# LiChaiUSTC/Speech-enhancement-based-on-a-maximum-likelihood-criterion

Hardware: AMD Instinct MI355X
Metric: training frames/sec (128-frame minibatch) (higher is better)
Workload: dtype f32

## Files before the change

### speech-enhancement-based-on-a-maximum-likelihood-criterion_amd/csrc/engine.hip

```cpp
#include <hip/hip_runtime.h>
#include <hip/hip_ext.h>

#include <dlfcn.h>
#include <math.h>
#include <stdarg.h>
#include <stdio.h>
#include <stdlib.h>
#include <string.h>

#include <algorithm>
#include <functional>
#include <mutex>
#include <string>
#include <vector>

#include "../../include/mlggd.h"
#include "../host/errmodel.h"
#include "kernels.hip.h"
#include "spectral.hip.h"
#include "score.hip.h"
#include "stoi.hip.h"
#include "stoi_rule.h"
#include "live.hip.h"
#include "live_rule.h"
// ... 545 lines not shown
                gather_arm(e);
            ProfScope ps(e, KC_FWD, l);
            FwdArgs fa = fwd_args(e, l, e->Y[l]);
            if (fwd64_used(e, l)) {
                fa.n_tiles = Np / 64;
                fa.b_tiles = e->Bp / 64;
                fa.b_shift = log2_or_minus1(fa.b_tiles);
                const size_t lds = t64_lds_floats() * sizeof(float);
                if (l != e->L - 1 && relu) {
                    CHK(ensure_lds(e, k_fwd64<FWD_RELU>, lds));
                    launch_timed(e, k_fwd64<FWD_RELU>, dim3(fa.n_tiles * fa.b_tiles), dim3(256), lds, e->stream, fa);
                } else if (l != e->L - 1) {
                    CHK(ensure_lds(e, k_fwd64<FWD_SIGMOID>, lds));
                    launch_timed(e, k_fwd64<FWD_SIGMOID>, dim3(fa.n_tiles * fa.b_tiles), dim3(256), lds, e->stream, fa);
                } else {
                    CHK(ensure_lds(e, k_fwd64<FWD_SLAB>, lds));
                    launch_timed(e, k_fwd64<FWD_SLAB>, dim3(fa.n_tiles * fa.b_tiles), dim3(256), lds, e->stream, fa);
                }
            } else if (l != e->L - 1) {
                long long *st = stamps_for(e, KC_FWD, l, n_tiles * b_tiles);
#define LAUNCH_FWD(NW, PIPE)                                                                                \
    {                                                                                                       \
        const size_t lds = fwd_lds_floats<NW, PIPE>() * sizeof(float);                                      \
        if (relu) {                                                                                         \
            CHK(ensure_lds(e, k_fwd<FWD_RELU, NW, PIPE>, lds));                                             \
            launch_timed(e, k_fwd<FWD_RELU, NW, PIPE>, dim3(n_tiles * b_tiles), dim3(64 * NW), lds, e->stream, fa, st); \
        } else {                                                                                            \
            CHK(ensure_lds(e, k_fwd<FWD_SIGMOID, NW, PIPE>, lds));                                          \
            launch_timed(e, k_fwd<FWD_SIGMOID, NW, PIPE>, dim3(n_tiles * b_tiles), dim3(64 * NW), lds, e->stream, fa, st); \
        }                                                                                                   \
    }
                if (e->fwd_nw == 16) LAUNCH_FWD(16, 0)
                else if (e->fwd_nw == 8 && e->fwd_pipe == 4) LAUNCH_FWD(8, 4)
                else if (e->fwd_nw == 8 && e->fwd_pipe) LAUNCH_FWD(8, 1)
                else if (e->fwd_nw == 8) LAUNCH_FWD(8, 0)
                else if (e->fwd_pipe == 4) LAUNCH_FWD(4, 4)
                else if (e->fwd_pipe) LAUNCH_FWD(4, 1)
                else LAUNCH_FWD(4, 0)
#undef LAUNCH_FWD
            } else {
                const int nwg = n_tiles * b_tiles * e->S_out;
                if (e->fwd_pipe == 4) {
                    const size_t lds = fwd_lds_floats<4, 4>() * sizeof(float);
                    CHK(ensure_lds(e, k_fwd<FWD_SLAB, 4, 4>, lds));
                    launch_timed(e, k_fwd<FWD_SLAB, 4, 4>, dim3(nwg), dim3(256), lds, e->stream, fa, (long long *)nullptr);
                } else {
                    const size_t lds = fwd_lds_floats<4, 1>() * sizeof(float);
                    launch_timed(e, k_fwd<FWD_SLAB, 4, 1>, dim3(nwg), dim3(256), lds, e->stream, fa, (long long *)nullptr);
                }
            }
        }
        CHK(launch_check("k_fwd"));
        if (cvscale) {
            const float keep = 1.0f - ((l == 1) ? e->cfg.visible_omit : e->cfg.hid_omit);
            hipLaunchKernelGGL(k_scale, dim3(1024), dim3(256), 0, e->stream, e->W[l], (size_t)Kp * Np, 1.0f / keep);
        }
        if (drop && l != e->L - 1) CHK(run_dropout(e, l, nullptr));
        if ((gather_flags & GATHER_HIDDEN_EACH) && l < e->L - 1) {
            CHK(gather_begin_armed(e));
            CHK(exchange_y(e, l, e->Y[l], nullptr));
            CHK(gather_end(e));
        }
// ... 51 lines not shown
    for (int j = 0; j < J.njobs && j < DWP_MAXJOBS; j++) {
        const DwpArgs &s = J.job[j];
        DwpArgs &a = key.job[j];
        a.Yrow = s.Yrow; a.dEdX = s.dEdX; a.Wt = s.Wt; a.delta = s.delta; a.G = s.G;
        a.bias = s.bias; a.dbias = s.dbias; a.gb = s.gb;
        a.ldA = s.ldA; a.K = s.K; a.N = s.N; a.Kp = s.Kp; a.Np = s.Np; a.n_wg = s.n_wg; a.ntiles = s.ntiles;
        a.k_first = s.k_first; a.wd_off = s.wd_off; a.do_bias = s.do_bias; a.k_base = s.k_base;
        key.tile_end[j] = J.tile_end[j];
    }
    key.njobs = J.njobs;
    key.total = J.total;
    for (const auto &t : e->dwp_tables)
        if (t.fused == fused && t.grid == grid && memcmp(&t.key, &key, sizeof(key)) == 0) {
            *out = t.dev;
            return MLGGD_OK;
        }
    if (e->dwp_tables.size() >= 64)
        return fail(MLGGD_ERR_STATE, "dW tile table: %zu launch plans cached and still missing -- plan key unstable",
                    e->dwp_tables.size());
    std::vector<DwpDesc> recs((size_t)J.total + 2 * (size_t)grid);
    size_t n = 0;
    for (int j = 0; j < J.njobs; j++) {
        const DwpArgs &a = J.job[j];
        for (int tl = 0; tl < a.ntiles; tl++, n++) {
            const int kt = a.k_first + tl / a.n_wg, nt = tl % a.n_wg;
            const int k0 = kt * 64, n0 = nt * 64;
            DwpDesc &d = recs[n];
            d.A = a.Yrow + (k0 - a.k_base);
            d.Bm = a.dEdX + n0;
            const size_t base = (size_t)k0 * a.Np + n0;
            int rows = a.K - k0;
            rows = rows < 0 ? 0 : rows > 64 ? 64 : rows;
            if (a.wd_off) {
                rows = 0;
                d.W = a.Wt;
                d.D = a.delta;
                d.szW = 0;
            } else {
                d.W = (fused ? a.Wt : a.G) + base;
                d.D = fused ? a.delta + base : nullptr;
                d.szW = (unsigned)(((size_t)a.Kp * a.Np - base) * sizeof(float));
            }
            const int colsw = a.Np - n0 < 64 ? a.Np - n0 : 64;
            int nbias = (a.do_bias && kt == 0) ? a.N - n0 : 0;
            nbias = nbias < 0 ? 0 : nbias > 64 ? 64 : nbias;
            d.bias = (fused ? a.bias : a.gb) + n0;
            d.dbias = fused ? a.dbias + n0 : nullptr;
            d.ldA = a.ldA;
            d.Np = a.Np;
            d.packed = (unsigned)rows | ((unsigned)colsw << 8) | ((unsigned)nbias << 16) | (1u << 24);
        }
    }
    if (n != (size_t)J.total) return fail(MLGGD_ERR_STATE, "dW tile table: %zu records for %d tiles", n, J.total);
    for (; n < recs.size(); n++) {
        DwpDesc &d = recs[n];
        d = recs[0];
        d.packed = 0;
        d.szW = 0;
    }
    mlggd_engine::DwpTable t;
    t.key = key;
    t.fused = fused;
    t.grid = grid;
    t.dev = nullptr;
// ... 26 lines not shown
        CHK(dwp_table(e, J, fused, grid, &table));
        unsigned nb;
        memcpy(&nb, &C.nf, sizeof(nb));
        if ((nb & 0x007FFFFFu) == 0u && C.nf >= 1.0f) {
            CHK(ensure_lds(e, k_dwp_bias<H, true>, lds));
            hipLaunchKernelGGL((k_dwp_bias<H, true>), dim3(grid), dim3(256), lds, st, table, J.total, C, (long long *)nullptr);
        } else {
            CHK(ensure_lds(e, k_dwp_bias<H, false>, lds));
            hipLaunchKernelGGL((k_dwp_bias<H, false>), dim3(grid), dim3(256), lds, st, table, J.total, C, (long long *)nullptr);
        }
        return launch_check("k_dwp_bias");
    }
    CHK(dwp_table(e, J, fused, grid, &table));
    if constexpr (H == 2 || H == 8) {
        if (e->stamp_class == KC_DW && e->stamp_layer == -1 && e->stamp_buf && fused && C.nf == 128.0f) {
            long long *sp = stamps_for(e, KC_DW, -1, 2 * grid);
            if (sp) {
                CHK(ensure_lds(e, k_dwp_phases<H>, lds));
                hipLaunchKernelGGL((k_dwp_phases<H>), dim3(grid), dim3(256), lds, st, table, J.total, C, sp);
                return launch_check("k_dwp_phases");
            }
        }
    }
    long long *stamps = stamps_for(e, KC_DW, stamp_layer, grid);
    if constexpr (H == 2) {
        static const int abl = getenv("MLGGD_DWP_ABLATE") ? atoi(getenv("MLGGD_DWP_ABLATE")) : 0;
        if (abl && fused) {
#define DWP_ABL(A_)                                                                                       \
    case A_:                                                                                              \
        CHK(ensure_lds(e, k_dwp_ablate<H, A_>, lds));                                                     \
        launch_timed(e, k_dwp_ablate<H, A_>, dim3(grid), dim3(256), lds, st, table, J.total, C, stamps);  \
        return launch_check("k_dwp_ablate");
            switch (abl) {
                DWP_ABL(1) DWP_ABL(2) DWP_ABL(3) DWP_ABL(4) DWP_ABL(7) DWP_ABL(15) DWP_ABL(31) DWP_ABL(63) DWP_ABL(16) DWP_ABL(48) DWP_ABL(256) DWP_ABL(512) DWP_ABL(576)
            default: return fail(MLGGD_ERR_ARG, "MLGGD_DWP_ABLATE=%d is not built", abl);
            }
#undef DWP_ABL
        }
    }
    unsigned nfbits;
    memcpy(&nfbits, &C.nf, sizeof(nfbits));
    const bool pow2 = (nfbits & 0x007FFFFFu) == 0u && C.nf >= 1.0f;
#define DWP_LAUNCH(FUSED_, POW2_)                                                                         \
    {                                                                                                     \
        CHK(ensure_lds(e, k_dwp<H, FUSED_, POW2_>, lds));                                                 \
        launch_timed(e, k_dwp<H, FUSED_, POW2_>, dim3(grid), dim3(256), lds, st, table, J.total, C, stamps); \
    }
    if (fused && pow2) DWP_LAUNCH(true, true)
    else if (fused) DWP_LAUNCH(true, false)
    else if (pow2) DWP_LAUNCH(false, true)
    else DWP_LAUNCH(false, false)
#undef DWP_LAUNCH
    return launch_check("k_dwp");
}
static bool dwp_usable(const mlggd_engine *e) {
    const int Hh = e->Bp / 64;
    return e->dw_persist && e->Bp % 64 == 0 && (Hh == 1 || Hh == 2 || Hh == 4 || Hh == 8);
}
static int launch_dwp(mlggd_engine *e, const DwpJobs &J, bool fused, hipStream_t st, int stamp_layer, int units = 0) {
    switch (units > 0 ? units : e->Bp / 64) {
    case 1: return launch_dwp_t<1>(e, J, fused, st, stamp_layer);
    case 2: return launch_dwp_t<2>(e, J, fused, st, stamp_layer);
    case 4: return launch_dwp_t<4>(e, J, fused, st, stamp_layer);
    case 8: return launch_dwp_t<8>(e, J, fused, st, stamp_layer);
    case 16: return launch_dwp_t<16>(e, J, fused, st, stamp_layer);
    default: return fail(MLGGD_ERR_STATE, "no dW kernel for %d units per tile", units);
    }
}

// ... 265 lines not shown
static int run_dx(mlggd_engine *e, int l) {
    const int Kp = e->lsp[l - 1], b_tiles = e->Bp / 32;
    const bool relu = e->cfg.activation == MLGGD_ACT_RELU;
    ProfScope ps(e, KC_DX, l);
    DxArgs xa = dx_args(e, l);
    if (dx64_used(e, l)) {
        xa.k_tiles = Kp / 64;
        xa.b_tiles = e->Bp / 64;
        xa.b_shift = log2_or_minus1(xa.b_tiles);
        const size_t lds = t64_lds_floats() * sizeof(float);
        if (relu) {
            CHK(ensure_lds(e, k_dx64<ACT_RELU>, lds));
            launch_timed(e, k_dx64<ACT_RELU>, dim3(xa.k_tiles * xa.b_tiles), dim3(256), lds, e->stream, xa);
        } else {
            CHK(ensure_lds(e, k_dx64<ACT_SIGMOID>, lds));
            launch_timed(e, k_dx64<ACT_SIGMOID>, dim3(xa.k_tiles * xa.b_tiles), dim3(256), lds, e->stream, xa);
        }
        return launch_check("k_dx64");
    }
    long long *st = stamps_for(e, KC_DX, l, (Kp / 32) * b_tiles);
#define LAUNCH_DX(NW, PIPE)                                                                                  \
    {                                                                                                        \
        const size_t lds = dx_lds_floats<NW, PIPE>() * sizeof(float);                                        \
        if (relu) {                                                                                          \
            CHK(ensure_lds(e, k_dx<NW, PIPE, ACT_RELU>, lds));                                               \
            launch_timed(e, k_dx<NW, PIPE, ACT_RELU>, dim3((Kp / 32) * b_tiles), dim3(64 * NW), lds, e->stream, xa, st); \
        } else {                                                                                             \
            CHK(ensure_lds(e, k_dx<NW, PIPE>, lds));                                                         \
            launch_timed(e, k_dx<NW, PIPE>, dim3((Kp / 32) * b_tiles), dim3(64 * NW), lds, e->stream, xa, st);  \
        }                                                                                                    \
    }
    const bool dma = e->dx_pipe == 4 && (Kp / 32) * b_tiles <= 256;
    if (e->dx_nw == 8 && e->dx_pipe) LAUNCH_DX(8, 1)
    else if (e->dx_nw == 8) LAUNCH_DX(8, 0)
    else if (dma) LAUNCH_DX(4, 4)
    else if (e->dx_pipe) LAUNCH_DX(4, 1)
    else LAUNCH_DX(4, 0)
#undef LAUNCH_DX
    return launch_check("k_dx");
}

static int launch_dw_layer(mlggd_engine *e, int l, const float *in_rows, bool fused, float nf, hipStream_t st) {
    const int Kp = e->lsp[l - 1], Np = e->lsp[l];
    const long tiles128 = (long)((Kp + 127) / 128) * ((Np + 127) / 128);
    const bool big = e->dw_tile == 0 ? tiles128 >= 192 : e->dw_tile == 2;
    ProfScope ps(e, KC_DW, l, st);
    if (dwp_usable(e)) return launch_dwp(e, dwp_jobs(e, l, l, in_rows, nf), fused, st, l);
    if (big) return launch_dw<2>(e, l, in_rows, fused, nf, st);
    return launch_dw<1>(e, l, in_rows, fused, nf, st);
}

static int launch_accum(float *dst, const float *a, const float *b, size_t n, hipStream_t st) {
    const size_t blocks = (n + 255) / 256;
    hipLaunchKernelGGL(k_accum, dim3((unsigned)(blocks > 2048 ? 2048 : blocks)), dim3(256), 0, st, dst, a, b, n);
    return launch_check("k_accum");
}

static size_t y_count(const mlggd_engine *e, int l) {
    return e->dp_a2a ? (size_t)e->world * e->Bp * e->shard_rows[l + 1] * 64 : (size_t)e->Bp * e->lsp[l];
}
static int keep_alloc(mlggd_engine *e) {
// ... 3281 lines not shown
```

### speech-enhancement-based-on-a-maximum-likelihood-criterion_amd/csrc/kernels.hip.h

```cpp
#pragma once
#include <hip/hip_runtime.h>
#include "nat_rule.h"

typedef float f32x16 __attribute__((ext_vector_type(16)));
typedef float f32x2 __attribute__((ext_vector_type(2)));

__device__ __forceinline__ f32x16 mfma32(float a, float b, f32x16 c) {
    return __builtin_amdgcn_mfma_f32_32x32x2f32(a, b, c, 0, 0, 0);
}
__device__ __forceinline__ int acc_row(int r, int lane) { return (r & 3) + 8 * (r >> 2) + 4 * (lane >> 5); }

__device__ __forceinline__ void divmod_by(int x, int d, int shift, int &q, int &r) {
    if (shift >= 0) {
        q = x >> shift;
        r = x & (d - 1);
    } else {
        q = (int)((unsigned)x / (unsigned)d);
        r = x - q * d;
    }
}
__device__ __forceinline__ void tile_of_block(int id, int u_tiles, int b_tiles, int b_shift, int &ut, int &bt, int map = 0) {
    if ((u_tiles & 7) == 0 && map != 2) {
        const int xcd = id & 7, slot = id >> 3;
        int q;
// ... 161 lines not shown
    const float *W, *Yt_in, *bias;
    float *Yt_out, *Y_out, *slab;
    int Kp, Np, Bp, N, n_tiles, b_tiles, S, map;
    int b_shift, s_shift;
    int yblk;
};
__device__ __forceinline__ size_t y_blocked_base(int u0, int yblk, int Bp) {
    const int blk = (int)((unsigned)u0 / (unsigned)yblk);
    return (size_t)blk * Bp * yblk + (u0 - blk * yblk);
}
template <int NW, int PIPE> constexpr int fwd_lds_floats() { return NW * (PIPE == 4 ? 4096 : 2048) + 32 * 36; }

template <int MODE, int NW, int PIPE = 1>
__device__ __forceinline__ void fwd_body(const FwdArgs &A, const int bid, float *smem, long long *stamps) {
    const float *__restrict__ W = A.W, *__restrict__ Yt_in = A.Yt_in, *__restrict__ bias = A.bias;
    float *__restrict__ Yt_out = A.Yt_out, *__restrict__ Y_out = A.Y_out, *__restrict__ slab = A.slab;
    const int Kp = A.Kp, Np = A.Np, Bp = A.Bp, N = A.N, n_tiles = A.n_tiles, b_tiles = A.b_tiles, S = A.S;
    float(*tileT)[36] = reinterpret_cast<float(*)[36]>(smem + NW * (PIPE == 4 ? 4096 : 2048));
    stamp(stamps, 0, bid);
    stamp_clk(stamps, 4, bid);
    const int tid = threadIdx.x, lane = tid & 63, wave = wave_id();
    const int i = lane & 31, h = lane >> 5;
    int id = bid, s = 0;
    if (MODE == FWD_SLAB) divmod_by(bid, S, A.s_shift, id, s);
    int nt, bt;
    tile_of_block(id, n_tiles, b_tiles, A.b_shift, nt, bt, A.map);
    const int n0 = nt * 32, b0 = bt * 32;

    const int P = Kp >> 1;
    const int slot = s * NW + wave, nslots = S * NW;
    int p0, p1;
    if (MODE == FWD_SLAB) {
        p0 = (int)((unsigned)(P * slot) / (unsigned)nslots);
        p1 = (int)((unsigned)(P * (slot + 1)) / (unsigned)nslots);
    } else {
        p0 = (int)((unsigned)(P * wave) / (unsigned)NW);
        p1 = (int)((unsigned)(P * (wave + 1)) / (unsigned)NW);
    }
    const int npairs = p1 - p0;
    const int nch = (npairs + 15) >> 4;

    const rsrc_t rW = make_rsrc(W, (size_t)Kp * Np * 4), rY = make_rsrc(Yt_in, (size_t)Kp * Bp * 4);
    const int r8 = lane >> 3, c4 = lane & 7;
    const int voW = (r8 * Np + n0 + 4 * c4) * 4, voY = (r8 * Bp + b0 + 4 * c4) * 4;
    float *stg = smem + wave * 2048;
    float *wdst = stg + r8 * 32 + 4 * c4;
// ... 830 lines not shown
    float *dbias;
    int ldA, Np;
    unsigned packed;
    unsigned szW;
};
static_assert(sizeof(DwpDesc) == 64, "four 16-byte quarters per record");
struct DwpRaw {
    unsigned w[16];
};
typedef unsigned u32x4 __attribute__((ext_vector_type(4)));
__device__ __forceinline__ DwpDesc dwp_decode(u32x4 v) {
    DwpRaw r;
#pragma unroll
    for (int q = 0; q < 4; q++)
#pragma unroll
        for (int c = 0; c < 4; c++) r.w[4 * q + c] = (unsigned)__builtin_amdgcn_readlane((int)v[c], q);
    return __builtin_bit_cast(DwpDesc, r);
}
struct DwpConst {
    int B;
    float nf, mom, lr, wc;
};

template <int H, bool FUSED, bool POW2, bool PHASES = false, int ABL = 0>
__device__ __forceinline__ void dwp_body(const DwpDesc *__restrict__ table, const int total, const DwpConst C, const int bid,
                                         const int nblocks, float *lds, long long *stamps) {
    stamp_clk(stamps, 0, bid);
    const int B = C.B;
    const float nf = C.nf, mom = C.mom, lr = C.lr, wc = C.wc;
    const float inv_nf = 1.0f / nf;
    constexpr int OOB = 0x7FFFFF00;
    const int tid = threadIdx.x, lane = tid & 63, wave = wave_id();
    const int i = lane & 31, h5 = lane >> 5;
    const int wm = wave >> 1, wn = wave & 1;
    const int scol = tid & 15, srow = tid >> 4;
    const int ec = lane & 7, er = lane >> 3;

    f32x16 acc, accp;
#pragma unroll
    for (int r = 0; r < 16; r++) acc[r] = accp[r] = 0.0f;
    float4 ra[4], rb[4];
    float4 pw0[4], pd0[4], pw1[4], pd1[4];
#pragma unroll
    for (int q = 0; q < 4; q++) pw1[q] = pd1[q] = make_float4(0.f, 0.f, 0.f, 0.f);
    float bsum = 0.0f, bsum_p = 0.0f;

    int t = bid;
    if (t >= total) return;
    const rsrc_t rT = make_rsrc(table, ((size_t)total + 2 * (size_t)nblocks) * sizeof(DwpDesc));
    const int voT = 16 * (lane & 3);
#define DWP_FETCH(TI) __builtin_bit_cast(u32x4, __builtin_amdgcn_raw_buffer_load_b128(rT, voT, (TI) * 64, 0))
    DwpDesc tc = dwp_decode(DWP_FETCH(t)), tn = dwp_decode(DWP_FETCH(t + nblocks)), tp = tc;
    tp.packed = 0;
    tp.szW = 0;
    u32x4 tnn_raw;

#define DWP_ROWS(T) ((int)((T).packed & 0xFFu))
#define DWP_COLS(T) ((int)(((T).packed >> 8) & 0xFFu))
#define DWP_NBIAS(T) ((int)(((T).packed >> 16) & 0xFFu))
#define DWP_SZAB(T) ((((T).packed >> 24) & 1u) ? 0x7FFFFFFFu : 0u)
#define DWP_DIVN(x) (POW2 ? (x) * inv_nf : (x) / nf)
#define DWP_DIVN2(x) (POW2 ? (x) * inv2 : (x) / nf2)
    const f32x2 mom2 = {mom, mom}, lr2 = {lr, lr}, wc2 = {wc, wc}, inv2 = {inv_nf, inv_nf}, nf2 = {nf, nf}, one2 = {1.0f, 1.0f};
#define DWP_OFF(T, IT)                                                                          \
    (((32 * wm + er + 8 * (IT)) < DWP_ROWS(T) && (32 * wn + 4 * ec) < DWP_COLS(T))               \
         ? ((32 * wm + er + 8 * (IT)) * T.Np + 32 * wn + 4 * ec) * 4                            \
         : OOB)
#define DWP_WRITE_UNIT(BUF)                                                                     \
    {                                                                                           \
        float *as = lds + (BUF)*8192, *bs = as + 4096;                                          \
        _Pragma("unroll") for (int q = 0; q < 4; q++) {                                         \
            *reinterpret_cast<float4 *>(as + (srow + 16 * q) * 64 + 4 * scol) = ra[q];          \
            *reinterpret_cast<float4 *>(bs + (srow + 16 * q) * 64 + 4 * scol) = rb[q];          \
        }                                                                                       \
    }
#define DWP_BIAS(BUF, HH)                                                                       \
    {                                                                                           \
        if (tid < DWP_NBIAS(tc)) {                                                              \
            const float *col = lds + (BUF)*8192 + 4096 + tid;                                   \
            int bend = B - 64 * (HH);                                                           \
            bend = bend < 64 ? bend : 64;                                                       \
            int b = 0;                                                                          \
            if ((HH) == 0 && bend > 0) {                                                        \
                bsum = col[0];                                                                  \
                b = 1;                                                                          \
            }                                                                                   \
            for (; b + 16 <= bend; b += 16) {                                                   \
                float v[16];                                                                    \
                _Pragma("unroll") for (int u = 0; u < 16; u++) v[u] = col[(b + u) * 64];        \
                _Pragma("unroll") for (int u = 0; u < 16; u++) bsum += v[u];                    \
            }                                                                                   \
            for (; b < bend; b++) bsum += col[b * 64];                                          \
        }                                                                                       \
    }
#define DWP_BIAS_UPDATE()                                                                       \
    {                                                                                           \
        if (tid < DWP_NBIAS(tp)) {                                                              \
            const rsrc_t rb_ = make_rsrc(tp.bias, 256), rdb_ = make_rsrc(tp.dbias, FUSED ? 256 : 0); \
            if (FUSED) {                                                                        \
                const float bv = bload(rb_, tid * 4, 0);                                        \
                const float d = mom * bload(rdb_, tid * 4, 0) - lr * (DWP_DIVN(bsum_p) + 0.0f * bv); \
                bstore1(d, rdb_, tid * 4);                                                      \
                bstore1(d + 1.0f * bv, rb_, tid * 4);                                           \
            } else {                                                                            \
                bstore1(bsum_p, rb_, tid * 4);                                                  \
            }                                                                                   \
        }                                                                                       \
    }
#define DWP_EPI_SCRATCH_WRITE(SB, R0, R1)                                                       \
    {                                                                                           \
        float *Tw = lds + (SB)*8192 + wave * 256;                                               \
        _Pragma("unroll") for (int r = (R0); r < (R1); r++) {                                   \
            const int kl = acc_row(r, lane);                                                    \
            Tw[(kl >> 3) * 1024 + ((kl >> 1) & 3) * 64 + (kl & 1) * 32 + i] = accp[r];          \
        }                                                                                       \
    }
#define DWP_EPI_SCRATCH_READ(SB, IT)                                                            \
    {                                                                                           \
        gq[IT] = *reinterpret_cast<const float4 *>(lds + (SB)*8192 + wave * 256 + (IT)*1024 + (er >> 1) * 64 + (er & 1) * 32 + 4 * ec); \
        asm volatile("" ::: "memory");                                                          \
    }
#define DWP_EPI_UPDATE(PW, PD, IT)                                                              \
    {                                                                                           \
        const float4 gv_ = gq[IT];                                                              \
        const int off = DWP_OFF(tp, IT);                                                        \
        if (FUSED && (ABL & 256)) {         \
            const float4 w = PW[IT];                                                            \
            float4 d = PD[IT];                                                                  \
            d.x = mom * d.x - lr * (DWP_DIVN(gv_.x) + wc * w.x);                                \
            d.y = mom * d.y - lr * (DWP_DIVN(gv_.y) + wc * w.y);                                \
            d.z = mom * d.z - lr * (DWP_DIVN(gv_.z) + wc * w.z);                                \
            d.w = mom * d.w - lr * (DWP_DIVN(gv_.w) + wc * w.w);                                \
            bstore4(d, rDp, off);                                                               \
            bstore4(make_float4(d.x + 1.0f * w.x, d.y + 1.0f * w.y, d.z + 1.0f * w.z, d.w + 1.0f * w.w), rWp, off); \
        } else if (FUSED) {  \
            const f32x2 w0 = {PW[IT].x, PW[IT].y}, w1 = {PW[IT].z, PW[IT].w};                   \
            f32x2 d0 = {PD[IT].x, PD[IT].y}, d1 = {PD[IT].z, PD[IT].w};                         \
            const f32x2 g0 = {gv_.x, gv_.y}, g1 = {gv_.z, gv_.w};                               \
            d0 = mom2 * d0 - lr2 * (DWP_DIVN2(g0) + wc2 * w0);                                  \
            d1 = mom2 * d1 - lr2 * (DWP_DIVN2(g1) + wc2 * w1);                                  \
            const f32x2 n0 = d0 + one2 * w0, n1 = d1 + one2 * w1;                               \
            bstore4(make_float4(d0.x, d0.y, d1.x, d1.y), rDp, off);                             \
            bstore4(make_float4(n0.x, n0.y, n1.x, n1.y), rWp, off);                             \
        } else {                                                                                \
            bstore4(gv_, rWp, off);                                                             \
        }                                                                                       \
    }
    long long ph_sum[5] = {0, 0, 0, 0, 0}, ph_last = 0;
#define DWP_PHASE(K)                                                                            \
    {                                                                                           \
        if (PHASES) {                                                                           \
            __builtin_amdgcn_sched_barrier(0);                                                  \
            const long long now_ = (long long)__builtin_amdgcn_s_memtime();                     \
            ph_sum[K] += now_ - ph_last;                                                        \
            ph_last = now_;                                                                     \
            __builtin_amdgcn_sched_barrier(0);                                                  \
        }                                                                                       \
    }
#define DWP_UNIT(HH, BUF, PW, PD)                                                               \
    {                                                                                           \
        const bool FIRSTU = (HH) == 0, LASTU = (HH) == H - 1;  \
        DWP_BIAS(BUF, HH)                                                                       \
        if (FIRSTU) DWP_BIAS_UPDATE()                                                           \
                                        \
        const rsrc_t rA_ = LASTU ? make_rsrc(tn.A, DWP_SZAB(tn)) : make_rsrc(tc.A, DWP_SZAB(tc)); \
        const rsrc_t rB_ = LASTU ? make_rsrc(tn.Bm, DWP_SZAB(tn)) : make_rsrc(tc.Bm, DWP_SZAB(tc)); \
        const int ldA_ = LASTU ? tn.ldA : tc.ldA, ldB_ = LASTU ? tn.Np : tc.Np;                 \
        const int row0_ = LASTU ? 0 : 64 * ((HH) + 1);                                          \
        const rsrc_t rWn = make_rsrc(tn.W, tn.szW), rDn = make_rsrc(tn.D, FUSED ? tn.szW : 0);  \
        const rsrc_t rWp = make_rsrc(tp.W, tp.szW), rDp = make_rsrc(tp.D, FUSED ? tp.szW : 0);  \
        const float *ap = lds + (BUF)*8192 + h5 * 64 + 32 * wm + i;                             \
        const float *bp = lds + (BUF)*8192 + 4096 + h5 * 64 + 32 * wn + i;                      \
        float fa[32], fb[32];                               \
        float4 gq[4];                                                                           \
        _Pragma("unroll") for (int p = 0; p < 4; p++) {                                         \
            fa[p] = (ABL & 8) ? 1.0f : ap[p * 128];                                             \
            fb[p] = (ABL & 8) ? 1.0f : bp[p * 128];                                             \
        }                                                                                       \
        if (FIRSTU) tnn_raw = DWP_FETCH(t + 2 * nblocks);                                       \
        __builtin_amdgcn_sched_barrier(0);                                                      \
        _Pragma("unroll") for (int g = 0; g < 16; g++) {                                        \
            if (!(ABL & 12)) {                                                                  \
                acc = mfma32(fa[2 * g], fb[2 * g], acc);                                        \
                acc = mfma32(fa[2 * g + 1], fb[2 * g + 1], acc);                                \
            } else if (!(ABL & 8)) {                                                            \
                asm volatile("" ::"v"(fa[2 * g]), "v"(fb[2 * g]), "v"(fa[2 * g + 1]), "v"(fb[2 * g + 1])); \
            }                                                                                   \
            if (g < 14 && !(ABL & 8)) {                                                         \
                _Pragma("unroll") for (int p = 2 * g + 4; p < 2 * g + 6; p++) {                 \
                    fa[p] = ap[p * 128];                                                        \
                    fb[p] = bp[p * 128];                                                        \
                }                                                                               \
            }                                                                                   \
                      \
                                \
            if (!(ABL & 512) && !(ABL & 16)) {                                                  \
                const int qa = FIRSTU ? g - 6 : g, qb = FIRSTU ? g : g - 4;                     \
                if (qa >= 0 && qa < 4) {                                                        \
                    float *dst = lds + ((BUF) ^ 1) * 8192 + (4 * wave + 16 * qa) * 64;          \
                    __builtin_amdgcn_raw_ptr_buffer_load_lds(rA_, (__attribute__((address_space(3))) void *)dst, 16, \
                                                             ((row0_ + srow + 16 * qa) * ldA_ + 4 * scol) * 4, 0, 0, 0); \
                }                                                                               \
                if (qb >= 0 && qb < 4) {                                                        \
                    float *dst = lds + ((BUF) ^ 1) * 8192 + 4096 + (4 * wave + 16 * qb) * 64;   \
                    __builtin_amdgcn_raw_ptr_buffer_load_lds(rB_, (__attribute__((address_space(3))) void *)dst, 16, \
                                                             ((row0_ + srow + 16 * qb) * ldB_ + 4 * scol) * 4, 0, 0, 0); \
                }                                                                               \
            }                                                                                   \
            if ((ABL & 512) && !(ABL & 16) && (FIRSTU ? g < 4 : g < 8)) {                        \
                const bool two_ = FIRSTU;                                                       \
                const int q = two_ ? g : g >> 1, row = row0_ + srow + 16 * q;                    \
                if (two_ || (g & 1) == 0) ra[q] = bload4(rA_, (row * ldA_ + 4 * scol) * 4, 0);   \
                if (two_ || (g & 1) == 1) rb[q] = bload4(rB_, (row * ldB_ + 4 * scol) * 4, 0);   \
            }                                                                                   \
             \
            if (FIRSTU) {                                                                       \
                if (g == 0) DWP_EPI_SCRATCH_WRITE((BUF) ^ 1, 0, 8)                              \
                if (g == 1) {                                                                   \
                    DWP_EPI_SCRATCH_WRITE((BUF) ^ 1, 8, 16)                                     \
                    __builtin_amdgcn_wave_barrier();                                            \
                }                                                                               \
                if (g >= 2 && g <= 5) DWP_EPI_SCRATCH_READ((BUF) ^ 1, g - 2)                    \
                if (g >= 4 && g <= 10 && (g & 1) == 0 && !(ABL & 1)) DWP_EPI_UPDATE(PW, PD, (g - 4) >> 1) \
            }                                                                                   \
                                                                                    \
            if (FUSED && LASTU && !(ABL & 2)) {                                                 \
                if (FIRSTU) {                                                                   \
                    if (g >= 12) {                                                              \
                        PW[g - 12] = bload4(rWn, DWP_OFF(tn, g - 12), 0);                       \
                        PD[g - 12] = bload4(rDn, DWP_OFF(tn, g - 12), 0);                       \
                    }                                                                           \
                } else if (g >= 8) {                                                            \
                    if (g < 12) PW[g - 8] = bload4(rWn, DWP_OFF(tn, g - 8), 0);                 \
                    else PD[g - 12] = bload4(rDn, DWP_OFF(tn, g - 12), 0);                      \
                }                                                                               \
            }                                                                                   \
             \
            if ((ABL & 512) && !(ABL & (32 | 64)) && g >= 12) {                                 \
                float *as_ = lds + ((BUF) ^ 1) * 8192, *bs_ = as_ + 4096;                       \
                *reinterpret_cast<float4 *>(as_ + (srow + 16 * (g - 12)) * 64 + 4 * scol) = ra[g - 12]; \
                *reinterpret_cast<float4 *>(bs_ + (srow + 16 * (g - 12)) * 64 + 4 * scol) = rb[g - 12]; \
            }                                                                                   \
            __builtin_amdgcn_sched_barrier(0);                                                  \
        }                                                                                       \
        DWP_PHASE(LASTU ? 2 : 0)                                                                \
        if ((ABL & 64) && !(ABL & 32)) DWP_WRITE_UNIT((BUF) ^ 1)                                \
        if (!(ABL & 512)) {                                                                     \
                             \
            constexpr int lo_ = 0;                                                              \
            const int younger = FIRSTU ? ((FUSED ? 2 : 1) + ((LASTU && FUSED) ? 8 : 0)) : ((LASTU && FUSED) ? 8 : 0); \
            if (younger == 0) __builtin_amdgcn_s_waitcnt(0x0F70 | lo_);                         \
            else if (younger == 1) __builtin_amdgcn_s_waitcnt(0x0F71);                          \
            else if (younger == 2) __builtin_amdgcn_s_waitcnt(0x0F72);                          \
            else if (younger == 8) __builtin_amdgcn_s_waitcnt(0x0F78);                          \
            else if (younger == 9) __builtin_amdgcn_s_waitcnt(0x0F79);                          \
            else __builtin_amdgcn_s_waitcnt(0x0F7A);                                            \
        }                                                                                       \
        __syncthreads();                                                                        \
        DWP_PHASE(LASTU ? 4 : 1)                                                                \
    }
#define DWP_TILE(BASE, PW, PD)                                                                  \
    {                                                                                           \
        _Pragma("unroll") for (int hh = 0; hh < H; hh++) DWP_UNIT(hh, ((BASE) + hh) & 1, PW, PD) \
         \
        accp = acc;                                                                             \
        _Pragma("unroll") for (int r = 0; r < 16; r++) acc[r] = 0.0f;                           \
        bsum_p = bsum;                                                                          \
        tp = tc;                                                                                \
        t += nblocks;                                                                           \
        if (t >= total) break;                                                                  \
        tc = tn;                                                                                \
        tn = dwp_decode(tnn_raw);                                                               \
    }

    {
        const rsrc_t rA_ = make_rsrc(tc.A, DWP_SZAB(tc)), rB_ = make_rsrc(tc.Bm, DWP_SZAB(tc));
        const rsrc_t rWc = make_rsrc(tc.W, tc.szW), rDc = make_rsrc(tc.D, FUSED ? tc.szW : 0);
#pragma unroll
        for (int q = 0; q < 4; q++) {
            const int row = srow + 16 * q;
            ra[q] = bload4(rA_, (row * tc.ldA + 4 * scol) * 4, 0);
            rb[q] = bload4(rB_, (row * tc.Np + 4 * scol) * 4, 0);
        }
#pragma unroll
        for (int q = 0; q < 4; q++) {
            pw0[q] = FUSED ? bload4(rWc, DWP_OFF(tc, q), 0) : make_float4(0.f, 0.f, 0.f, 0.f);
            pd0[q] = FUSED ? bload4(rDc, DWP_OFF(tc, q), 0) : make_float4(0.f, 0.f, 0.f, 0.f);
        }
    }
    DWP_WRITE_UNIT(0)
    __syncthreads();
    if (PHASES) ph_last = (long long)__builtin_amdgcn_s_memtime();
    bool last_set1 = true;
    for (;;) {
        last_set1 = false;
        DWP_TILE(0, pw1, pd1)
        last_set1 = true;
        DWP_TILE(H & 1, pw0, pd0)
    }
    {
        DWP_BIAS_UPDATE()
        const rsrc_t rWp = make_rsrc(tp.W, tp.szW), rDp = make_rsrc(tp.D, FUSED ? tp.szW : 0);
        float4 gq[4];
        DWP_EPI_SCRATCH_WRITE(0, 0, 16)
        __builtin_amdgcn_wave_barrier();
        _Pragma("unroll") for (int it = 0; it < 4; it++) DWP_EPI_SCRATCH_READ(0, it)
        if (last_set1) {
            _Pragma("unroll") for (int it = 0; it < 4; it++) DWP_EPI_UPDATE(pw1, pd1, it)
        } else {
            _Pragma("unroll") for (int it = 0; it < 4; it++) DWP_EPI_UPDATE(pw0, pd0, it)
        }
    }
    stamp_clk(stamps, 2, bid);
    if (stamps != nullptr && threadIdx.x == 0) stamps[(size_t)bid * 8 + 4] = (t - bid) / nblocks;
    if (PHASES && stamps != nullptr && threadIdx.x == 0) {
#pragma unroll
        for (int k = 0; k < 5; k++) stamps[(size_t)(nblocks + bid) * 8 + k] = ph_sum[k];
    }
#undef DWP_PHASE
#undef DWP_FETCH
#undef DWP_WRITE_UNIT
#undef DWP_OFF
#undef DWP_BIAS
#undef DWP_BIAS_UPDATE
#undef DWP_EPI_SCRATCH_WRITE
#undef DWP_EPI_SCRATCH_READ
#undef DWP_EPI_UPDATE
#undef DWP_UNIT
#undef DWP_TILE
#undef DWP_ROWS
#undef DWP_COLS
#undef DWP_NBIAS
#undef DWP_SZAB
#undef DWP_DIVN
#undef DWP_DIVN2
}

extern __shared__ __attribute__((aligned(16))) float g_dyn_lds[];

template <int MODE, int NW, int PIPE = 1>
__global__ __launch_bounds__(64 * NW) void k_fwd(FwdArgs A, long long *stamps) {
    fwd_body<MODE, NW, PIPE>(A, (int)blockIdx.x, g_dyn_lds, stamps);
}
template <int NW, int PIPE = 1, int ACT = ACT_SIGMOID>
__global__ __launch_bounds__(64 * NW) void k_dx(DxArgs A, long long *stamps) {
    dx_body<NW, PIPE, ACT>(A, (int)blockIdx.x, g_dyn_lds, stamps);
}
#include "kernels64.hip.h"
template <int H, bool FUSED, bool POW2>
__global__ __launch_bounds__(256) void k_dwp(const DwpDesc *__restrict__ table, int total, DwpConst C, long long *stamps) {
    dwp_body<H, FUSED, POW2>(table, total, C, (int)blockIdx.x, (int)gridDim.x, g_dyn_lds, stamps);
}
template <int H, bool POW2>
__global__ __launch_bounds__(256) void k_dwp_bias(const DwpDesc *__restrict__ table, int total, DwpConst C, long long *stamps) {
    dwp_body<H, true, POW2, false, 15>(table, total, C, (int)blockIdx.x, (int)gridDim.x, g_dyn_lds, stamps);
}
template <int H, int ABL>
__global__ __launch_bounds__(256) void k_dwp_ablate(const DwpDesc *__restrict__ table, int total, DwpConst C, long long *stamps) {
    dwp_body<H, true, true, false, ABL>(table, total, C, (int)blockIdx.x, (int)gridDim.x, g_dyn_lds, stamps);
}
template <int H>
__global__ __launch_bounds__(256) void k_dwp_phases(const DwpDesc *__restrict__ table, int total, DwpConst C, long long *stamps) {
    dwp_body<H, true, true, true>(table, total, C, (int)blockIdx.x, (int)gridDim.x, g_dyn_lds, stamps);
}
__global__ __launch_bounds__(256) void k_apply_update(float *__restrict__ Wt, float *__restrict__ delta,
                                                      const float *__restrict__ G, size_t n4, float nf, float mom,
                                                      float lr, float wc) {
    const size_t stride = (size_t)gridDim.x * blockDim.x;
    for (size_t idx = (size_t)blockIdx.x * blockDim.x + threadIdx.x; idx < n4; idx += stride) {
        const float4 g = reinterpret_cast<const float4 *>(G)[idx];
        float4 w = reinterpret_cast<float4 *>(Wt)[idx];
        float4 d = reinterpret_cast<float4 *>(delta)[idx];
        d.x = mom * d.x - lr * (g.x / nf + wc * w.x);
        d.y = mom * d.y - lr * (g.y / nf + wc * w.y);
        d.z = mom * d.z - lr * (g.z / nf + wc * w.z);
        d.w = mom * d.w - lr * (g.w / nf + wc * w.w);
        w.x = d.x + 1.0f * w.x;
        w.y = d.y + 1.0f * w.y;
        w.z = d.z + 1.0f * w.z;
        w.w = d.w + 1.0f * w.w;
        reinterpret_cast<float4 *>(delta)[idx] = d;
        reinterpret_cast<float4 *>(Wt)[idx] = w;
// ... 720 lines not shown
```

Before: 1.008 million.

## Specialise kernels on timing stamps and slim dW epilogue address math

```diff
diff --git a/speech-enhancement-based-on-a-maximum-likelihood-criterion_amd/csrc/engine.hip b/speech-enhancement-based-on-a-maximum-likelihood-criterion_amd/csrc/engine.hip
--- a/speech-enhancement-based-on-a-maximum-likelihood-criterion_amd/csrc/engine.hip
+++ b/speech-enhancement-based-on-a-maximum-likelihood-criterion_amd/csrc/engine.hip
@@ -591,13 +591,15 @@
 #define LAUNCH_FWD(NW, PIPE)                                                                                \
     {                                                                                                       \
         const size_t lds = fwd_lds_floats<NW, PIPE>() * sizeof(float);                                      \
-        if (relu) {                                                                                         \
-            CHK(ensure_lds(e, k_fwd<FWD_RELU, NW, PIPE>, lds));                                             \
-            launch_timed(e, k_fwd<FWD_RELU, NW, PIPE>, dim3(n_tiles * b_tiles), dim3(64 * NW), lds, e->stream, fa, st); \
-        } else {                                                                                            \
-            CHK(ensure_lds(e, k_fwd<FWD_SIGMOID, NW, PIPE>, lds));                                          \
-            launch_timed(e, k_fwd<FWD_SIGMOID, NW, PIPE>, dim3(n_tiles * b_tiles), dim3(64 * NW), lds, e->stream, fa, st); \
-        }                                                                                                   \
+        if (relu && st) LAUNCH_FWD_(FWD_RELU, NW, PIPE, true)                                               \
+        else if (relu) LAUNCH_FWD_(FWD_RELU, NW, PIPE, false)                                               \
+        else if (st) LAUNCH_FWD_(FWD_SIGMOID, NW, PIPE, true)                                               \
+        else LAUNCH_FWD_(FWD_SIGMOID, NW, PIPE, false)                                                      \
+    }
+#define LAUNCH_FWD_(MODE, NW, PIPE, STAMPED)                                                                \
+    {                                                                                                       \
+        CHK(ensure_lds(e, k_fwd<MODE, NW, PIPE, STAMPED>, lds));                                            \
+        launch_timed(e, k_fwd<MODE, NW, PIPE, STAMPED>, dim3(n_tiles * b_tiles), dim3(64 * NW), lds, e->stream, fa, st); \
     }
                 if (e->fwd_nw == 16) LAUNCH_FWD(16, 0)
                 else if (e->fwd_nw == 8 && e->fwd_pipe == 4) LAUNCH_FWD(8, 4)
@@ -607,6 +609,7 @@
                 else if (e->fwd_pipe) LAUNCH_FWD(4, 1)
                 else LAUNCH_FWD(4, 0)
 #undef LAUNCH_FWD
+#undef LAUNCH_FWD_
             } else {
                 const int nwg = n_tiles * b_tiles * e->S_out;
                 if (e->fwd_pipe == 4) {
@@ -704,6 +707,7 @@
     size_t n = 0;
     for (int j = 0; j < J.njobs; j++) {
         const DwpArgs &a = J.job[j];
+        if (a.Np >= (1 << 17)) return fail(MLGGD_ERR_ARG, "dW tile table: layer of %d units is too wide", a.Np);
         for (int tl = 0; tl < a.ntiles; tl++, n++) {
             const int kt = a.k_first + tl / a.n_wg, nt = tl % a.n_wg;
             const int k0 = kt * 64, n0 = nt * 64;
@@ -721,7 +725,9 @@
             } else {
                 d.W = (fused ? a.Wt : a.G) + base;
                 d.D = fused ? a.delta + base : nullptr;
-                d.szW = (unsigned)(((size_t)a.Kp * a.Np - base) * sizeof(float));
+                const size_t to_end = ((size_t)a.Kp * a.Np - base) * sizeof(float);
+                const size_t to_row = (size_t)rows * a.Np * sizeof(float);
+                d.szW = (unsigned)(to_end < to_row ? to_end : to_row);
             }
             const int colsw = a.Np - n0 < 64 ? a.Np - n0 : 64;
             int nbias = (a.do_bias && kt == 0) ? a.N - n0 : 0;
@@ -794,29 +800,34 @@
             }
         }
     }
-    long long *stamps = stamps_for(e, KC_DW, stamp_layer, grid);
     if constexpr (H == 2) {
         static const int abl = getenv("MLGGD_DWP_ABLATE") ? atoi(getenv("MLGGD_DWP_ABLATE")) : 0;
         if (abl && fused) {
 #define DWP_ABL(A_)                                                                                       \
     case A_:                                                                                              \
         CHK(ensure_lds(e, k_dwp_ablate<H, A_>, lds));                                                     \
-        launch_timed(e, k_dwp_ablate<H, A_>, dim3(grid), dim3(256), lds, st, table, J.total, C, stamps);  \
+        launch_timed(e, k_dwp_ablate<H, A_>, dim3(grid), dim3(256), lds, st, table, J.total, C, (long long *)nullptr); \
         return launch_check("k_dwp_ablate");
             switch (abl) {
-                DWP_ABL(1) DWP_ABL(2) DWP_ABL(3) DWP_ABL(4) DWP_ABL(7) DWP_ABL(15) DWP_ABL(31) DWP_ABL(63) DWP_ABL(16) DWP_ABL(48) DWP_ABL(256) DWP_ABL(512) DWP_ABL(576)
+                DWP_ABL(1) DWP_ABL(2) DWP_ABL(3) DWP_ABL(4) DWP_ABL(7) DWP_ABL(15) DWP_ABL(31) DWP_ABL(63) DWP_ABL(16) DWP_ABL(48) DWP_ABL(256) DWP_ABL(1024) DWP_ABL(2048) DWP_ABL(512) DWP_ABL(576)
             default: return fail(MLGGD_ERR_ARG, "MLGGD_DWP_ABLATE=%d is not built", abl);
             }
 #undef DWP_ABL
         }
     }
+    long long *stamps = stamps_for(e, KC_DW, stamp_layer, grid);
     unsigned nfbits;
     memcpy(&nfbits, &C.nf, sizeof(nfbits));
     const bool pow2 = (nfbits & 0x007FFFFFu) == 0u && C.nf >= 1.0f;
 #define DWP_LAUNCH(FUSED_, POW2_)                                                                         \
     {                                                                                                     \
-        CHK(ensure_lds(e, k_dwp<H, FUSED_, POW2_>, lds));                                                 \
-        launch_timed(e, k_dwp<H, FUSED_, POW2_>, dim3(grid), dim3(256), lds, st, table, J.total, C, stamps); \
+        if (stamps) {                                                                                     \
+            CHK(ensure_lds(e, k_dwp<H, FUSED_, POW2_, true>, lds));                                       \
+            launch_timed(e, k_dwp<H, FUSED_, POW2_, true>, dim3(grid), dim3(256), lds, st, table, J.total, C, stamps); \
+        } else {                                                                                          \
+            CHK(ensure_lds(e, k_dwp<H, FUSED_, POW2_>, lds));                                             \
+            launch_timed(e, k_dwp<H, FUSED_, POW2_>, dim3(grid), dim3(256), lds, st, table, J.total, C, stamps); \
+        }                                                                                                 \
     }
     if (fused && pow2) DWP_LAUNCH(true, true)
     else if (fused) DWP_LAUNCH(true, false)
@@ -1128,13 +1139,15 @@
 #define LAUNCH_DX(NW, PIPE)                                                                                  \
     {                                                                                                        \
         const size_t lds = dx_lds_floats<NW, PIPE>() * sizeof(float);                                        \
-        if (relu) {                                                                                          \
-            CHK(ensure_lds(e, k_dx<NW, PIPE, ACT_RELU>, lds));                                               \
-            launch_timed(e, k_dx<NW, PIPE, ACT_RELU>, dim3((Kp / 32) * b_tiles), dim3(64 * NW), lds, e->stream, xa, st); \
-        } else {                                                                                             \
-            CHK(ensure_lds(e, k_dx<NW, PIPE>, lds));                                                         \
-            launch_timed(e, k_dx<NW, PIPE>, dim3((Kp / 32) * b_tiles), dim3(64 * NW), lds, e->stream, xa, st);  \
-        }                                                                                                    \
+        if (relu && st) LAUNCH_DX_(NW, PIPE, ACT_RELU, true)                                                 \
+        else if (relu) LAUNCH_DX_(NW, PIPE, ACT_RELU, false)                                                 \
+        else if (st) LAUNCH_DX_(NW, PIPE, ACT_SIGMOID, true)                                                 \
+        else LAUNCH_DX_(NW, PIPE, ACT_SIGMOID, false)                                                        \
+    }
+#define LAUNCH_DX_(NW, PIPE, ACT, STAMPED)                                                                   \
+    {                                                                                                        \
+        CHK(ensure_lds(e, k_dx<NW, PIPE, ACT, STAMPED>, lds));                                               \
+        launch_timed(e, k_dx<NW, PIPE, ACT, STAMPED>, dim3((Kp / 32) * b_tiles), dim3(64 * NW), lds, e->stream, xa, st); \
     }
     const bool dma = e->dx_pipe == 4 && (Kp / 32) * b_tiles <= 256;
     if (e->dx_nw == 8 && e->dx_pipe) LAUNCH_DX(8, 1)
@@ -1143,6 +1156,7 @@
     else if (e->dx_pipe) LAUNCH_DX(4, 1)
     else LAUNCH_DX(4, 0)
 #undef LAUNCH_DX
+#undef LAUNCH_DX_
     return launch_check("k_dx");
 }
 
diff --git a/speech-enhancement-based-on-a-maximum-likelihood-criterion_amd/csrc/kernels.hip.h b/speech-enhancement-based-on-a-maximum-likelihood-criterion_amd/csrc/kernels.hip.h
--- a/speech-enhancement-based-on-a-maximum-likelihood-criterion_amd/csrc/kernels.hip.h
+++ b/speech-enhancement-based-on-a-maximum-likelihood-criterion_amd/csrc/kernels.hip.h
@@ -207,6 +207,9 @@
     const int tid = threadIdx.x, lane = tid & 63, wave = wave_id();
     const int i = lane & 31, h = lane >> 5;
     int id = bid, s = 0;
+    if (MODE == FWD_SLAB)
+        asm volatile("" ::"s"(W), "s"(Yt_in), "s"(slab), "s"(Kp), "s"(Np), "s"(Bp), "s"(N), "s"(n_tiles), "s"(b_tiles), "s"(S),
+                     "s"(A.map), "s"(A.b_shift), "s"(A.s_shift));
     if (MODE == FWD_SLAB) divmod_by(bid, S, A.s_shift, id, s);
     int nt, bt;
     tile_of_block(id, n_tiles, b_tiles, A.b_shift, nt, bt, A.map);
@@ -1083,6 +1086,7 @@
     float nf, mom, lr, wc;
 };
 
+constexpr int DWP_UPDATE_FORM = 2048;
 template <int H, bool FUSED, bool POW2, bool PHASES = false, int ABL = 0>
 __device__ __forceinline__ void dwp_body(const DwpDesc *__restrict__ table, const int total, const DwpConst C, const int bid,
                                          const int nblocks, float *lds, long long *stamps) {
@@ -1090,7 +1094,7 @@
     const int B = C.B;
     const float nf = C.nf, mom = C.mom, lr = C.lr, wc = C.wc;
     const float inv_nf = 1.0f / nf;
-    constexpr int OOB = 0x7FFFFF00;
+    constexpr unsigned OOB = 0x7F000000u;
     const int tid = threadIdx.x, lane = tid & 63, wave = wave_id();
     const int i = lane & 31, h5 = lane >> 5;
     const int wm = wave >> 1, wn = wave & 1;
@@ -1107,26 +1111,24 @@
     float bsum = 0.0f, bsum_p = 0.0f;
 
     int t = bid;
-    if (t >= total) return;
     const rsrc_t rT = make_rsrc(table, ((size_t)total + 2 * (size_t)nblocks) * sizeof(DwpDesc));
     const int voT = 16 * (lane & 3);
 #define DWP_FETCH(TI) __builtin_bit_cast(u32x4, __builtin_amdgcn_raw_buffer_load_b128(rT, voT, (TI) * 64, 0))
-    DwpDesc tc = dwp_decode(DWP_FETCH(t)), tn = dwp_decode(DWP_FETCH(t + nblocks)), tp = tc;
+    u32x4 tc_raw = DWP_FETCH(t), tn_raw = DWP_FETCH(t + nblocks), tp_raw = tc_raw, tnn_raw;
+    DwpDesc tc = dwp_decode(tc_raw), tn = dwp_decode(tn_raw), tp = tc;
     tp.packed = 0;
     tp.szW = 0;
-    u32x4 tnn_raw;
-
-#define DWP_ROWS(T) ((int)((T).packed & 0xFFu))
+
 #define DWP_COLS(T) ((int)(((T).packed >> 8) & 0xFFu))
 #define DWP_NBIAS(T) ((int)(((T).packed >> 16) & 0xFFu))
 #define DWP_SZAB(T) ((((T).packed >> 24) & 1u) ? 0x7FFFFFFFu : 0u)
 #define DWP_DIVN(x) (POW2 ? (x) * inv_nf : (x) / nf)
 #define DWP_DIVN2(x) (POW2 ? (x) * inv2 : (x) / nf2)
-    const f32x2 mom2 = {mom, mom}, lr2 = {lr, lr}, wc2 = {wc, wc}, inv2 = {inv_nf, inv_nf}, nf2 = {nf, nf}, one2 = {1.0f, 1.0f};
-#define DWP_OFF(T, IT)                                                                          \
-    (((32 * wm + er + 8 * (IT)) < DWP_ROWS(T) && (32 * wn + 4 * ec) < DWP_COLS(T))               \
-         ? ((32 * wm + er + 8 * (IT)) * T.Np + 32 * wn + 4 * ec) * 4                            \
-         : OOB)
+    f32x2 mom2 = {mom, mom}, lr2 = {lr, lr}, wc2 = {wc, wc}, inv2 = {inv_nf, inv_nf}, nf2 = {nf, nf}, one2 = {1.0f, 1.0f};
+    constexpr int UPD = (ABL & (256 | 1024 | 2048)) ? (ABL & (256 | 1024 | 2048)) : DWP_UPDATE_FORM;
+    if (UPD == 1024) asm volatile("" : "+v"(mom2), "+v"(lr2), "+v"(wc2), "+v"(inv2), "+v"(nf2), "+v"(one2));
+#define DWP_OFF0(T) ((32 * wn + 4 * ec) < DWP_COLS(T) ? (unsigned)(((32 * wm + er) * T.Np + 32 * wn + 4 * ec) * 4) : OOB)
+#define DWP_OFF(BASE, T, IT) ((int)((BASE) + (unsigned)((IT) * 32 * T.Np)))
 #define DWP_WRITE_UNIT(BUF)                                                                     \
     {                                                                                           \
         float *as = lds + (BUF)*8192, *bs = as + 4096;                                          \
@@ -1141,23 +1143,26 @@
             const float *col = lds + (BUF)*8192 + 4096 + tid;                                   \
             int bend = B - 64 * (HH);                                                           \
             bend = bend < 64 ? bend : 64;                                                       \
+                                                     \
+            asm volatile("" : "+s"(bend));                                                      \
             int b = 0;                                                                          \
-            if ((HH) == 0 && bend > 0) {                                                        \
+            if ((HH) == 0) {  \
                 bsum = col[0];                                                                  \
                 b = 1;                                                                          \
             }                                                                                   \
-            for (; b + 16 <= bend; b += 16) {                                                   \
+            _Pragma("clang loop unroll(disable)") for (; b + 16 <= bend; b += 16) {             \
                 float v[16];                                                                    \
                 _Pragma("unroll") for (int u = 0; u < 16; u++) v[u] = col[(b + u) * 64];        \
                 _Pragma("unroll") for (int u = 0; u < 16; u++) bsum += v[u];                    \
             }                                                                                   \
-            for (; b < bend; b++) bsum += col[b * 64];                                          \
+            _Pragma("clang loop unroll(disable)") for (; b < bend; b++) bsum += col[b * 64];    \
         }                                                                                       \
     }
 #define DWP_BIAS_UPDATE()                                                                       \
     {                                                                                           \
         if (tid < DWP_NBIAS(tp)) {                                                              \
-            const rsrc_t rb_ = make_rsrc(tp.bias, 256), rdb_ = make_rsrc(tp.dbias, FUSED ? 256 : 0); \
+            const DwpDesc tb_ = dwp_decode(tp_raw);                                             \
+            const rsrc_t rb_ = make_rsrc(tb_.bias, 256), rdb_ = make_rsrc(tb_.dbias, FUSED ? 256 : 0); \
             if (FUSED) {                                                                        \
                 const float bv = bload(rb_, tid * 4, 0);                                        \
                 const float d = mom * bload(rdb_, tid * 4, 0) - lr * (DWP_DIVN(bsum_p) + 0.0f * bv); \
@@ -1184,8 +1189,8 @@
 #define DWP_EPI_UPDATE(PW, PD, IT)                                                              \
     {                                                                                           \
         const float4 gv_ = gq[IT];                                                              \
-        const int off = DWP_OFF(tp, IT);                                                        \
-        if (FUSED && (ABL & 256)) {         \
+        const int off = DWP_OFF(offp_, tp, IT);                                                 \
+        if (FUSED && UPD == 256) {                     \
             const float4 w = PW[IT];                                                            \
             float4 d = PD[IT];                                                                  \
             d.x = mom * d.x - lr * (DWP_DIVN(gv_.x) + wc * w.x);                                \
@@ -1228,8 +1233,11 @@
         const rsrc_t rB_ = LASTU ? make_rsrc(tn.Bm, DWP_SZAB(tn)) : make_rsrc(tc.Bm, DWP_SZAB(tc)); \
         const int ldA_ = LASTU ? tn.ldA : tc.ldA, ldB_ = LASTU ? tn.Np : tc.Np;                 \
         const int row0_ = LASTU ? 0 : 64 * ((HH) + 1);                                          \
+                \
+        const int voA_ = (srow * ldA_ + 4 * scol) * 4, voB_ = (srow * ldB_ + 4 * scol) * 4;     \
         const rsrc_t rWn = make_rsrc(tn.W, tn.szW), rDn = make_rsrc(tn.D, FUSED ? tn.szW : 0);  \
         const rsrc_t rWp = make_rsrc(tp.W, tp.szW), rDp = make_rsrc(tp.D, FUSED ? tp.szW : 0);  \
+        const unsigned offp_ = FIRSTU ? DWP_OFF0(tp) : 0u, offn_ = (FUSED && LASTU) ? DWP_OFF0(tn) : 0u; \
         const float *ap = lds + (BUF)*8192 + h5 * 64 + 32 * wm + i;                             \
         const float *bp = lds + (BUF)*8192 + 4096 + h5 * 64 + 32 * wn + i;                      \
         float fa[32], fb[32];                               \
@@ -1260,12 +1268,12 @@
                 if (qa >= 0 && qa < 4) {                                                        \
                     float *dst = lds + ((BUF) ^ 1) * 8192 + (4 * wave + 16 * qa) * 64;          \
                     __builtin_amdgcn_raw_ptr_buffer_load_lds(rA_, (__attribute__((address_space(3))) void *)dst, 16, \
-                                                             ((row0_ + srow + 16 * qa) * ldA_ + 4 * scol) * 4, 0, 0, 0); \
+                                                             voA_, (row0_ + 16 * qa) * ldA_ * 4, 0, 0);  \
                 }                                                                               \
                 if (qb >= 0 && qb < 4) {                                                        \
                     float *dst = lds + ((BUF) ^ 1) * 8192 + 4096 + (4 * wave + 16 * qb) * 64;   \
                     __builtin_amdgcn_raw_ptr_buffer_load_lds(rB_, (__attribute__((address_space(3))) void *)dst, 16, \
-                                                             ((row0_ + srow + 16 * qb) * ldB_ + 4 * scol) * 4, 0, 0, 0); \
+                                                             voB_, (row0_ + 16 * qb) * ldB_ * 4, 0, 0);  \
                 }                                                                               \
             }                                                                                   \
             if ((ABL & 512) && !(ABL & 16) && (FIRSTU ? g < 4 : g < 8)) {                        \
@@ -1288,12 +1296,12 @@
             if (FUSED && LASTU && !(ABL & 2)) {                                                 \
                 if (FIRSTU) {                                                                   \
                     if (g >= 12) {                                                              \
-                        PW[g - 12] = bload4(rWn, DWP_OFF(tn, g - 12), 0);                       \
-                        PD[g - 12] = bload4(rDn, DWP_OFF(tn, g - 12), 0);                       \
+                        PW[g - 12] = bload4(rWn, DWP_OFF(offn_, tn, g - 12), 0);                \
+                        PD[g - 12] = bload4(rDn, DWP_OFF(offn_, tn, g - 12), 0);                \
                     }                                                                           \
                 } else if (g >= 8) {                                                            \
-                    if (g < 12) PW[g - 8] = bload4(rWn, DWP_OFF(tn, g - 8), 0);                 \
-                    else PD[g - 12] = bload4(rDn, DWP_OFF(tn, g - 12), 0);                      \
+                    if (g < 12) PW[g - 8] = bload4(rWn, DWP_OFF(offn_, tn, g - 8), 0);          \
+                    else PD[g - 12] = bload4(rDn, DWP_OFF(offn_, tn, g - 12), 0);               \
                 }                                                                               \
             }                                                                                   \
              \
@@ -1328,15 +1336,19 @@
         _Pragma("unroll") for (int r = 0; r < 16; r++) acc[r] = 0.0f;                           \
         bsum_p = bsum;                                                                          \
         tp = tc;                                                                                \
+        tp_raw = tc_raw;                                                                        \
         t += nblocks;                                                                           \
         if (t >= total) break;                                                                  \
         tc = tn;                                                                                \
+        tc_raw = tn_raw;                                                                        \
         tn = dwp_decode(tnn_raw);                                                               \
+        tn_raw = tnn_raw;                                                                       \
     }
 
     {
         const rsrc_t rA_ = make_rsrc(tc.A, DWP_SZAB(tc)), rB_ = make_rsrc(tc.Bm, DWP_SZAB(tc));
         const rsrc_t rWc = make_rsrc(tc.W, tc.szW), rDc = make_rsrc(tc.D, FUSED ? tc.szW : 0);
+        const unsigned offc_ = DWP_OFF0(tc);
 #pragma unroll
         for (int q = 0; q < 4; q++) {
             const int row = srow + 16 * q;
@@ -1345,8 +1357,8 @@
         }
 #pragma unroll
         for (int q = 0; q < 4; q++) {
-            pw0[q] = FUSED ? bload4(rWc, DWP_OFF(tc, q), 0) : make_float4(0.f, 0.f, 0.f, 0.f);
-            pd0[q] = FUSED ? bload4(rDc, DWP_OFF(tc, q), 0) : make_float4(0.f, 0.f, 0.f, 0.f);
+            pw0[q] = FUSED ? bload4(rWc, DWP_OFF(offc_, tc, q), 0) : make_float4(0.f, 0.f, 0.f, 0.f);
+            pd0[q] = FUSED ? bload4(rDc, DWP_OFF(offc_, tc, q), 0) : make_float4(0.f, 0.f, 0.f, 0.f);
         }
     }
     DWP_WRITE_UNIT(0)
@@ -1362,6 +1374,7 @@
     {
         DWP_BIAS_UPDATE()
         const rsrc_t rWp = make_rsrc(tp.W, tp.szW), rDp = make_rsrc(tp.D, FUSED ? tp.szW : 0);
+        const unsigned offp_ = DWP_OFF0(tp);
         float4 gq[4];
         DWP_EPI_SCRATCH_WRITE(0, 0, 16)
         __builtin_amdgcn_wave_barrier();
@@ -1382,6 +1395,7 @@
 #undef DWP_FETCH
 #undef DWP_WRITE_UNIT
 #undef DWP_OFF
+#undef DWP_OFF0
 #undef DWP_BIAS
 #undef DWP_BIAS_UPDATE
 #undef DWP_EPI_SCRATCH_WRITE
@@ -1389,7 +1403,6 @@
 #undef DWP_EPI_UPDATE
 #undef DWP_UNIT
 #undef DWP_TILE
-#undef DWP_ROWS
 #undef DWP_COLS
 #undef DWP_NBIAS
 #undef DWP_SZAB
@@ -1399,26 +1412,26 @@
 
 extern __shared__ __attribute__((aligned(16))) float g_dyn_lds[];
 
-template <int MODE, int NW, int PIPE = 1>
+template <int MODE, int NW, int PIPE = 1, bool STAMPED = false>
 __global__ __launch_bounds__(64 * NW) void k_fwd(FwdArgs A, long long *stamps) {
-    fwd_body<MODE, NW, PIPE>(A, (int)blockIdx.x, g_dyn_lds, stamps);
-}
-template <int NW, int PIPE = 1, int ACT = ACT_SIGMOID>
+    fwd_body<MODE, NW, PIPE>(A, (int)blockIdx.x, g_dyn_lds, STAMPED ? stamps : nullptr);
+}
+template <int NW, int PIPE = 1, int ACT = ACT_SIGMOID, bool STAMPED = false>
 __global__ __launch_bounds__(64 * NW) void k_dx(DxArgs A, long long *stamps) {
-    dx_body<NW, PIPE, ACT>(A, (int)blockIdx.x, g_dyn_lds, stamps);
+    dx_body<NW, PIPE, ACT>(A, (int)blockIdx.x, g_dyn_lds, STAMPED ? stamps : nullptr);
 }
 #include "kernels64.hip.h"
-template <int H, bool FUSED, bool POW2>
+template <int H, bool FUSED, bool POW2, bool STAMPED = false>
 __global__ __launch_bounds__(256) void k_dwp(const DwpDesc *__restrict__ table, int total, DwpConst C, long long *stamps) {
-    dwp_body<H, FUSED, POW2>(table, total, C, (int)blockIdx.x, (int)gridDim.x, g_dyn_lds, stamps);
+    dwp_body<H, FUSED, POW2>(table, total, C, (int)blockIdx.x, (int)gridDim.x, g_dyn_lds, STAMPED ? stamps : nullptr);
 }
 template <int H, bool POW2>
 __global__ __launch_bounds__(256) void k_dwp_bias(const DwpDesc *__restrict__ table, int total, DwpConst C, long long *stamps) {
-    dwp_body<H, true, POW2, false, 15>(table, total, C, (int)blockIdx.x, (int)gridDim.x, g_dyn_lds, stamps);
+    dwp_body<H, true, POW2, false, 15>(table, total, C, (int)blockIdx.x, (int)gridDim.x, g_dyn_lds, nullptr);
 }
 template <int H, int ABL>
 __global__ __launch_bounds__(256) void k_dwp_ablate(const DwpDesc *__restrict__ table, int total, DwpConst C, long long *stamps) {
-    dwp_body<H, true, true, false, ABL>(table, total, C, (int)blockIdx.x, (int)gridDim.x, g_dyn_lds, stamps);
+    dwp_body<H, true, true, false, ABL>(table, total, C, (int)blockIdx.x, (int)gridDim.x, g_dyn_lds, nullptr);
 }
 template <int H>
 __global__ __launch_bounds__(256) void k_dwp_phases(const DwpDesc *__restrict__ table, int total, DwpConst C, long long *stamps) {
```

Result: faster. 1.024 million, median of 6 (+1.6%).
